# tsunrise/r1cs-spartan

Measured on AMD Instinct MI355X. Metric: R1CS constraints proved/sec at 2^20, higher is better.
Workload: dtype bls12-381 Fr/Fq Montgomery (u32 limbs)

## Files before the change

r1cs-spartan_amd/csrc/msm_common.hip:

```cpp
#include "msm_common.hpp"

#include <algorithm>
#include <cmath>
#include <cstring>
#include <cstdlib>

namespace spx {

__device__ __constant__ constexpr uint32_t kFqR2[12] = {0x1c341746u, 0xf4df1f34u, 0x09d104f1u, 0x0a76e6a6u,
                                                       0x4c95b6d5u, 0x8de5476cu, 0x939d83c0u, 0x67eb88a9u,
                                                       0xb519952du, 0x9a793e85u, 0x92cae3aau, 0x11988fe5u};

struct Digits {
    uint32_t s[8];
    uint32_t carry = 0;
    DEV int32_t next(uint32_t c) {
        const uint32_t full = 1u << c, half = full >> 1;
        uint32_t v = (s[0] & (full - 1)) + carry;
#pragma unroll
        for (int k = 0; k < 7; ++k) s[k] = (s[k] >> c) | (s[k + 1] << (32 - c));
        s[7] >>= c;
        carry = v > half;
        return carry ? (int32_t)v - (int32_t)full : (int32_t)v;
    }
// ... 390 lines not shown
    if (!handoff_last(ticket, g.nbin, &last)) return;
    for (int l = 0; l <= nlev; ++l) {
        uint32_t carry = 0;
        const uint32_t* src = binsum + (size_t)l * (g.nbin + 1);
        uint32_t* dst = binpfx + (size_t)l * (g.nbin + 1);
        for (uint32_t b = 0; b < g.nbin; b += NT) {
            const uint32_t i = b + f;
            const uint32_t x = i < g.nbin ? ld_agent(src + i) : 0u;
            const uint32_t e = block_excl_scan<NT>(x, agg, L.sh);
            if (i < g.nbin) dst[i] = carry + e;
            carry += agg;
        }
        if (f == 0) dst[g.nbin] = carry;
    }
    if (f == 0) *ticket = 0u;
}

__global__ __launch_bounds__(kScanThreads) void k_sort_final(SortGeom g, int nlev, LevPtrs lev, const uint32_t* __restrict__ binpfx) {
    const uint64_t t = blockIdx.x * (uint64_t)kScanThreads + threadIdx.x;
    const uint32_t l = (uint32_t)(t / (g.nb + 1)), b = (uint32_t)(t % (g.nb + 1));
    if ((int)l > nlev) return;
    const uint32_t* pf = binpfx + (size_t)l * (g.nbin + 1);
    lev.p[l][b] = b < g.nb ? lev.p[l][b] + pf[b >> g.sb] : pf[g.nbin];
}

uint32_t seg1_len(bool) { return kSeg1Default; }

uint32_t seg1_fit(uint32_t seg1, uint64_t refs, int waves_per_simd, int lanes_per_elem) {
    static const int cus = [] {
        int dev = 0, n = 0;
        if (hipGetDevice(&dev) != hipSuccess || hipDeviceGetAttribute(&n, hipDeviceAttributeMultiprocessorCount, dev) != hipSuccess)
            n = 0;
        return n;
    }();
    if (cus <= 0 || refs == 0) return seg1;
    const uint64_t slots = (uint64_t)cus * 4 * waves_per_simd * 64 / lanes_per_elem;
    const uint64_t nthr = (refs + seg1 - 1) / seg1;
    const uint64_t rounds = (nthr + slots - 1) / slots;
    if (rounds > 16) return seg1;
    const uint64_t fit = (refs + rounds * slots - 1) / (rounds * slots);
    return (uint32_t)std::min<uint64_t>(seg1, std::max<uint64_t>(fit, std::min<uint32_t>(seg1, 8)));
}

MsmWorkspace* msm_ws_create() {
    auto* ws = new MsmWorkspace();
    ws->hot_on = msm_hot_default();
    return ws;
}
void msm_ws_destroy(MsmWorkspace* ws) { delete ws; }
void msm_ws_staging_reset(MsmWorkspace* ws) {
    if (ws) ws->pin.reset();
}
void msm_ws_note_overflow(MsmWorkspace* ws) {
    if (ws) ws->cap_scale = std::min(ws->cap_scale * 1.5, 64.0);
}
void msm_ws_set_hot(MsmWorkspace* ws, bool on) {
    if (ws) ws->hot_on = on;
}
bool msm_hot_default() {
    static const bool v = [] {
        const char* e = getenv("SPX_MSM_HOT");
        return !(e && atoi(e) == 0 && *e);
    }();
    return v;
}
uint32_t msm_hot_cap(uint64_t tot_refs, uint32_t seg1, int nlev) {
    uint64_t per = 1;
    for (int l = 0; l <= nlev; ++l) per *= kSeg;
    const uint64_t cap = tot_refs / ((per - 1) * std::max<uint32_t>(seg1, 1)) + 1;
    if (cap < tot_refs / (per * std::max<uint32_t>(seg1, 1)) + 1) throw std::runtime_error("MSM: hot-bucket list capacity");
    return (uint32_t)std::min<uint64_t>(cap, 0xffffffffu);
}

static double msm_cap_env() {
    const char* e = getenv("SPX_MSM_CAP_SCALE");
    const double v = e ? atof(e) : 1.0;
    return v > 0 ? v : 1.0;
}

MsmPlan msm_plan(const MsmInst* ih, int ninst, const MsmShard& sh, double cap_scale) {
    MsmPlan o;
    const int G = std::max(1, sh.world);
    int g = 0;
    while ((1 << g) < G) ++g;
    if ((1 << g) != G || sh.rank < 0 || sh.rank >= G) throw std::runtime_error("MSM shard: bad rank / world");
    o.compact = G > 1 && !sh.dense;
    uint64_t tot_refs = 0;
    double split_refs = 0, whole_refs = 0;
    int nsplit = 0;
    for (int i = 0; i < ninst; ++i) {
        MsmInst I = ih[i];
        if (!I.size) continue;
        if (I.c < 3 || I.c > 24) throw std::runtime_error("MSM window bits out of range");
        if (I.W < msm_windows(I.c)) throw std::runtime_error("MSM: too few windows for the window bits");
        const uint32_t lbf = I.c - 1;
        if (G > 1 && (int)lbf - g >= 2) {
            I.lb = lbf - g;
            I.lg = (uint32_t)g;
            I.sel = (uint32_t)sh.rank;
            split_refs += (double)I.size * I.W / G;
            ++nsplit;
        } else if (i % G == sh.rank) {
            I.lb = lbf;
            I.lg = 0;
            I.sel = 0;
            whole_refs += (double)I.size * I.W;
        } else {
            continue;
        }
        I.out = (uint32_t)i;
        I.bucket_off = o.nb;
        I.ref_off = (uint32_t)tot_refs;
        o.nb += 1u << I.lb;
        o.prefix.push_back(o.tot_sc);
        o.tot_sc += I.size;
        tot_refs += (uint64_t)I.size * I.W;
        o.mu_max = std::max(o.mu_max, (double)I.size * I.W / (double)(1u << lbf));
        o.any_split |= I.lg != 0;
        o.insts.push_back(I);
    }
    const int nact = (int)o.insts.size();
    o.prefix.push_back(o.tot_sc);
    if (tot_refs >= 0xffffffffull) throw std::runtime_error("MSM batch too large");
    if (o.compact) {
        const double cap = whole_refs + (split_refs + 8.0 * std::sqrt(split_refs) + 2048.0 * nsplit) * cap_scale * msm_cap_env();
        tot_refs = std::min<uint64_t>(tot_refs, (uint64_t)std::ceil(cap));
    }
    o.tot_refs = tot_refs;
    o.node_off.resize(nact);
    o.cnt.resize(nact);
    uint32_t tot_nodes = 0;
    for (int i = 0; i < nact; ++i) {
        o.node_off[i] = tot_nodes;
        const int lg = (int)o.insts[i].lb - (int)std::min<uint32_t>(kTreeChunkLog, o.insts[i].lb - 1);
        o.cnt[i] = 1u << lg;
        tot_nodes += o.cnt[i];
        o.levels = std::max(o.levels, lg);
    }
    o.wp.assign((size_t)(o.levels + 1) * (nact + 1), 0);
    o.cin.assign((size_t)(o.levels + 1) * nact, 0);
    uint32_t maxc = 1;
    for (int i = 0; i < nact; ++i) maxc = std::max(maxc, o.cnt[i]);
    o.top_from = o.levels + 1;
    for (int lv = 0; lv <= o.levels; ++lv) {
        uint64_t acc = 0;
        for (int i = 0; i < nact; ++i) {
            uint32_t nin = lv == 0 ? (o.cnt[i] * 2) : std::max(1u, o.cnt[i] >> (lv - 1));
            uint32_t nout = lv == 0 ? o.cnt[i] : std::max(1u, o.cnt[i] >> lv);
            o.cin[(size_t)lv * nact + i] = nin;
            o.wp[(size_t)lv * (nact + 1) + i] = acc;
            acc += nout;
        }
        o.wp[(size_t)lv * (nact + 1) + nact] = acc;
        if (lv >= 1 && o.top_from > o.levels && std::max(1u, maxc >> (lv - 1)) <= kTopNodes) o.top_from = lv;
    }
    return o;
}

void msm_upload_plan(MsmWorkspace* ws, MsmPlan& p, hipStream_t s) {
    const int nact = (int)p.insts.size();
    auto al = [](size_t x) { return (x + 15) & ~(size_t)15; };
    const size_t b0 = al(sizeof(MsmInst) * nact), b1 = al(8 * p.prefix.size()), b2 = al(8 * p.wp.size()),
                 b3 = al(4 * p.cin.size()), b4 = al(4 * p.node_off.size());
    std::vector<uint8_t> h(b0 + b1 + b2 + b3 + b4, 0);
    size_t o = 0;
    memcpy(h.data() + o, p.insts.data(), sizeof(MsmInst) * nact), o += b0;
    memcpy(h.data() + o, p.prefix.data(), 8 * p.prefix.size()), o += b1;
    memcpy(h.data() + o, p.wp.data(), 8 * p.wp.size()), o += b2;
    memcpy(h.data() + o, p.cin.data(), 4 * p.cin.size()), o += b3;
    memcpy(h.data() + o, p.node_off.data(), 4 * p.node_off.size());
    uint8_t* d = (uint8_t*)ws->tables.ensure(h.size());
    HIPCHK(hipMemcpyAsync(d, ws->pin.stage(h.data(), h.size()), h.size(), hipMemcpyHostToDevice, s));
    p.d_insts = (MsmInst*)d;
    p.d_prefix = (uint64_t*)(d + b0);
    p.d_wp = (uint64_t*)(d + b0 + b1);
    p.d_cin = (uint32_t*)(d + b0 + b1 + b2);
    p.d_noff = (uint32_t*)(d + b0 + b1 + b2 + b3);
}

static constexpr double kStagedRho = 6.0;
static constexpr size_t kTicketBytes = 128;
static int sort_form_env() {
    static const int v = [] {
        const char* e = getenv("SPX_SORT_FORM");
        if (!e) return -1;
        return std::string(e) == "staged" ? 1 : std::string(e) == "direct" ? 0 : -1;
    }();
    return v;
}
static SortGeom sort_geom(const MsmPlan& p, bool& staged) {
    SortGeom g;
    g.nb = p.nb;
    g.tot_sc = p.tot_sc;
    const double rho = p.tot_sc ? (double)p.tot_refs / (double)p.tot_sc : 0.0;
    staged = sort_form_env() >= 0 ? sort_form_env() == 1 : rho >= kStagedRho;
    int lnb = 0;
    while ((1ull << lnb) < p.nb) ++lnb;
    int sb = 8;
    if (staged)
        while (sb > 0 && (double)(1u << sb) * std::max(p.mu_max, 1.0) > 0.8 * kBinStage) --sb;
    else
        sb = std::min(8, std::max(0, lnb - 9));
    while (sb < 8 && ((uint64_t)p.nb + (1u << sb) - 1) >> sb > kMaxBins) ++sb;
    g.sb = (uint32_t)sb;
    g.nbin = (p.nb + (1u << g.sb) - 1) >> g.sb;
    if (g.nbin > kMaxBins) throw std::runtime_error("MSM batch: too many buckets for the sort");
    const int threads = staged ? kTileThreads : kDirectThreads, tiles_log = staged ? 8 : 9;
    const uint64_t tile_sc = (uint64_t)threads << tiles_log;
    g.spt = (uint32_t)std::min<uint64_t>(64, std::max<uint64_t>(1, (p.tot_sc + tile_sc - 1) / tile_sc));
    const uint64_t ts = (uint64_t)threads * g.spt;
    const uint64_t nt = (p.tot_sc + ts - 1) / ts;
    if (nt > 0x7fffffffull / kSub) throw std::runtime_error("MSM batch: too many tiles");
    g.ntile = (uint32_t)std::max<uint64_t>(1, nt);
    g.sub = staged ? kSub : 1;
    return g;
}

MsmSorted msm_sort(MsmWorkspace* ws, const MsmPlan& p, const Fr* scalars, void* out_dev, size_t out_bytes, hipStream_t s,
                   uint32_t seg1, int nlev) {
    if (nlev > kMaxLev) throw std::runtime_error("MSM: too many partial levels");
    if (out_bytes % 4) throw std::runtime_error("MSM: output bytes not a multiple of 4");
    MsmSorted o;
    bool staged = false;
    const SortGeom g = sort_geom(p, staged);
    const uint32_t nb = p.nb;
    const uint64_t cap = std::max<uint64_t>(p.tot_refs, 1);
    uint32_t* st = (uint32_t*)((uint8_t*)out_dev + out_bytes - 16);
    o.offs = (uint32_t*)ws->offs.ensure(4 * (size_t)(nb + 1));
    o.refs = (uint32_t*)ws->refs.ensure(4 * cap);
    uint32_t* cnt = (uint32_t*)ws->cnt.ensure(4 * (size_t)g.nbin * g.ntile * g.sub);
    uint32_t* bintot = (uint32_t*)ws->bintot.ensure(4 * (size_t)g.nbin);
    uint32_t* binbase = (uint32_t*)ws->binbase.ensure(4 * (size_t)(g.nbin + 1));
    uint32_t* binsum = (uint32_t*)ws->binsum.ensure(4 * 2 * (size_t)(kMaxLev + 1) * (g.nbin + 1));
    uint32_t* binpfx = binsum + (size_t)(kMaxLev + 1) * (g.nbin + 1);
    uint32_t* sref = (uint32_t*)ws->stage_ref.ensure(4 * cap + 16);
    uint8_t* sfine = (uint8_t*)ws->stage_fine.ensure(cap + 16);
    uint32_t* lv = (uint32_t*)ws->lvl.ensure(4 * (size_t)(nb + 1) * (nlev + 1));
    uint32_t* tk = (uint32_t*)ws->tickets.ensure(kTicketBytes);
    if (!ws->tickets_zeroed) {
        HIPCHK(hipMemsetAsync(tk, 0, kTicketBytes, s));
        ws->tickets_zeroed = true;
    }
    LevPtrs lp{};
    for (int l = 0; l <= nlev; ++l) lp.p[l] = lv + (size_t)l * (nb + 1);
    o.hot_cap = msm_hot_cap(p.tot_refs, seg1, nlev);
    o.hot = (uint32_t*)ws->hot.ensure(4 * (size_t)o.hot_cap);
    const int nact = (int)p.insts.size();
    kp_begin(KP_SORT, s);
    hipLaunchKernelGGL(k_sort_count, dim3(g.ntile * g.sub), dim3(kCountThreads), 0, s, p.d_insts, p.d_prefix, nact, scalars, g,
                       cnt, (uint32_t*)out_dev, (uint32_t)(out_bytes / 4));
    const uint32_t cap32 = (uint32_t)std::min<uint64_t>(cap, 0xffffffffu);
    if (staged) {
        hipLaunchKernelGGL(k_sort_scan<kRowThreads>, dim3(g.nbin), dim3(kRowThreads), 0, s, cnt, g, bintot, binbase, tk, cap32,
                           st, o.offs + nb);
        hipLaunchKernelGGL(k_sort_scatter, dim3(g.ntile), dim3(kTileThreads), 0, s, p.d_insts, p.d_prefix, nact, scalars, g, cnt,
                           binbase, st, sref, sfine);
        hipLaunchKernelGGL((k_sort_bins<kBinThreads, kBinStage>), dim3(g.nbin), dim3(kBinThreads), 0, s, g, binbase, st, sref,
                           sfine, o.offs, o.refs, seg1, nlev, lp, binsum, binpfx, tk + 16, o.hot, o.hot_cap);
    } else {
        hipLaunchKernelGGL(k_sort_scan<kDirectThreads>, dim3(g.nbin), dim3(kDirectThreads), 0, s, cnt, g, bintot, binbase, tk,
                           cap32, st, o.offs + nb);
        hipLaunchKernelGGL(k_sort_scatter_direct, dim3(g.ntile), dim3(kDirectThreads), 0, s, p.d_insts, p.d_prefix, nact, scalars,
                           g, cnt, binbase, st, sref, sfine);
        hipLaunchKernelGGL((k_sort_bins<kDirectThreads, 0>), dim3(g.nbin), dim3(kDirectThreads), 0, s, g, binbase, st, sref,
                           sfine, o.offs, o.refs, seg1, nlev, lp, binsum, binpfx, tk + 16, o.hot, o.hot_cap);
    }
    const uint64_t nfin = (uint64_t)(nlev + 1) * (nb + 1);
    hipLaunchKernelGGL(k_sort_final, dim3((unsigned)((nfin + kScanThreads - 1) / kScanThreads)), dim3(kScanThreads), 0, s, g,
                       nlev, lp, binpfx);
    kp_end(64.0 * p.tot_sc + 14.0 * p.tot_refs + 16.0 * g.nbin * g.ntile * g.sub, s, (double)p.tot_refs);
    o.np_off = lp.p[0];
    for (int l = 1; l <= nlev; ++l) o.lev.push_back(lp.p[l]);
    return o;
}

DEV bool fq_canon_to_mont(Fq& r, const Fq& c) {
    uint32_t br = 0;
#pragma unroll
    for (int i = 0; i < 12; ++i) {
        uint64_t d = (uint64_t)c.v[i] - kFqP[i] - br;
        br = (uint32_t)(d >> 63);
    }
    Fq r2;
#pragma unroll
    for (int i = 0; i < 12; ++i) r2.v[i] = kFqR2[i];
    fe_mul(r, c, r2);
    return br != 0;
}

template <int NF>
__global__ void k_points_from_bytes(Fq* pts, uint64_t n, int* err) {
    for (uint64_t j = blockIdx.x * (uint64_t)blockDim.x + threadIdx.x; j < n; j += (uint64_t)gridDim.x * blockDim.x) {
        Fq* p = pts + j * NF;
        Fq last;
        load_vec(last, p + NF - 1);
        const uint32_t flags = last.v[11] >> 30;
        bool ok = true;
        if (flags & 1u) {
            Fq z;
            fe_zero(z);
#pragma unroll
            for (int k = 0; k < NF; ++k) store_vec(p + k, z);
            continue;
        }
        Fq m[NF];
#pragma unroll
        for (int k = 0; k < NF; ++k) {
// ... 64 lines not shown
```

r1cs-spartan_amd/csrc/msm_common.hpp:

```cpp
#pragma once
#include <algorithm>
#include <cstring>
#include <stdexcept>
#include <string>
#include <vector>

#include "kernels.hpp"

namespace spx {

static constexpr uint32_t kSeg1Default = 64;
uint32_t seg1_len(bool g2);
uint32_t seg1_fit(uint32_t seg1, uint64_t refs, int waves_per_simd, int lanes_per_elem);
static constexpr uint32_t kSeg = 4;
static constexpr uint32_t kTreeChunkLog = 2;
static constexpr uint32_t kTopNodes = 32;
static constexpr int kLight = 256;
static constexpr int kHeavy = 64;

#define HIPCHK(x)                                                                                     \
    do {                                                                                              \
        hipError_t e_ = (x);                                                                          \
        if (e_ != hipSuccess) throw std::runtime_error(std::string("HIP error: ") + hipGetErrorString(e_) + \
                                                       " at " __FILE__ ":" + std::to_string(__LINE__)); \
    } while (0)

template <class F>
DEV bool aff_is_sentinel(const Aff<F>& a) {
    return FieldOps<F>::is_zero(a.x) && FieldOps<F>::is_zero(a.y);
}
template <class F>
DEV void aff_set_sentinel(Aff<F>& a) {
    FieldOps<F>::zero(a.x);
    FieldOps<F>::zero(a.y);
}

DEV int find_slot(const uint64_t* prefix, int n, uint64_t g) {
    int lo = 0, hi = n - 1;
    while (lo < hi) {
        int mid = (lo + hi + 1) >> 1;
        if (prefix[mid] <= g)
            lo = mid;
        else
            hi = mid - 1;
    }
    return lo;
}
DEV uint32_t find_bucket(const uint32_t* off, uint32_t nb, uint32_t s) {
    uint32_t lo = 0, hi = nb - 1;
    while (lo < hi) {
        uint32_t mid = (lo + hi + 1) >> 1;
        if (off[mid] <= s)
            lo = mid;
        else
            hi = mid - 1;
    }
    return lo;
}


struct DBuf {
    void* p = nullptr;
    size_t cap = 0;
    void* ensure(size_t bytes) {
        if (bytes > cap) {
            if (p) HIPCHK(hipFree(p));
            size_t nb = std::max(bytes, cap + cap / 2);
            HIPCHK(hipMalloc(&p, nb));
            cap = nb;
        }
        return p;
    }
    ~DBuf() {
        if (p) (void)hipFree(p);
    }
};

struct PinArena {
    static constexpr size_t kCap = 512 << 10;
    uint8_t* p = nullptr;
    size_t used = 0;
    PinArena() { HIPCHK(hipHostMalloc((void**)&p, kCap)); }
    ~PinArena() {
        if (p) (void)hipHostFree(p);
    }
    template <class T>
    T* stage(const T* src, size_t count) {
        const size_t o = (used + 255) & ~(size_t)255, b = sizeof(T) * count;
        if (o + b > kCap) throw std::runtime_error("MSM pinned staging arena exhausted");
        used = o + b;
        memcpy(p + o, src, b);
        return (T*)(p + o);
    }
    void reset() { used = 0; }
};

struct MsmWorkspace {
    DBuf tables, offs, refs, pa, pb, tree_a, tree_b;
    DBuf cnt, bintot, binbase, binsum, stage_ref, stage_fine, lvl, tickets;
    bool tickets_zeroed = false;
    DBuf hot;
    bool hot_on = true;
    double cap_scale = 1.0;
    PinArena pin;
};

struct MsmPlan {
    std::vector<MsmInst> insts;
    std::vector<uint64_t> prefix;
    uint32_t nb = 0;
    uint64_t tot_sc = 0;
    uint64_t tot_refs = 0;
    bool compact = false;
    double mu_max = 0;
    bool any_split = false;
    std::vector<uint32_t> node_off, cnt;
    int levels = 0;
    int top_from = 1;
    std::vector<uint64_t> wp;
    std::vector<uint32_t> cin;
    MsmInst* d_insts = nullptr;
    uint64_t *d_prefix = nullptr, *d_wp = nullptr;
    uint32_t *d_cin = nullptr, *d_noff = nullptr;
};
MsmPlan msm_plan(const MsmInst* ih, int ninst, const MsmShard& sh, double cap_scale);
void msm_upload_plan(MsmWorkspace* ws, MsmPlan& p, hipStream_t s);

uint32_t msm_hot_cap(uint64_t tot_refs, uint32_t seg1, int nlev);
struct MsmSorted {
    uint32_t *offs, *refs, *np_off;
    std::vector<uint32_t*> lev;
    uint32_t* hot = nullptr;
    uint32_t hot_cap = 0;
};
MsmSorted msm_sort(MsmWorkspace* ws, const MsmPlan& p, const Fr* scalars, void* out_dev, size_t out_bytes, hipStream_t s,
                   uint32_t seg1, int nlev);

}
```

r1cs-spartan_amd/csrc/msm_impl.hpp:

```cpp
#pragma once
#include "curve29.hpp"
#include "fq2pair.hpp"
#include "msm_common.hpp"

namespace spx {

template <class F>
struct Acc;
struct AffRaw {
    Fq x, y;
};
template <>
struct Acc<Fq> {
    using Pt = G1Slot;
    using T = F29;
    using TA = F29;
    static constexpr int kLanes = 1, kWaves = 1;
    static DEV void ld_raw(AffRaw& a, const G1Slot* p) { load_vec(*(Aff<Fq>*)&a, &p->p); }
    static DEV void unpack(T& x, T& y, const AffRaw& a) {
        f29_unpack(x, a.x.v);
        f29_unpack(y, a.y.v);
    }
    static DEV void ld_aff(T& x, T& y, const G1Slot* p) {
        AffRaw a;
// ... 133 lines not shown
        else
            x29_set_inf(p);
        return;
    }
    T sq;
    O::sqr(sq, S2::sel(h, P, R));
    const T sqo = S2::swap(sq);
    const T PP = S2::sel(h, sq, sqo), Tr = S2::sel(h, sqo, sq);
    T m3;
    O::mul(m3, S2::sel(h, P, U1), PP);
    const T m3o = S2::swap(m3);
    const T PPP = S2::sel(h, m3, m3o), Q = S2::sel(h, m3o, m3);
    T w, t;
    O::template sub<2>(w, Tr, PPP);
    O::add(t, Q, Q);
    O::template sub<4>(w, w, t);
    O::template reduce<8>(w);
    O::template sub<2>(t, Q, w);
    T y4, z4;
    O::mul(y4, S2::sel(h, R, Sa), S2::sel(h, t, PPP));
    O::mul(z4, S2::sel(h, ZZ12, ZZZ12), S2::sel(h, PP, PPP));
    const T y4o = S2::swap(y4), z4o = S2::swap(z4);
    O::template sub<2>(p.y, S2::sel(h, y4, y4o), S2::sel(h, y4o, y4));
    O::template reduce<4>(p.y);
    p.x = w;
    p.zz = S2::sel(h, z4, z4o);
    p.zzz = S2::sel(h, z4o, z4);
}

template <class F>
struct TreeLanes {
    static constexpr int v = 2 * Acc<F>::kLanes;
};
template <class F>
DEV void tree_add(X29<typename Acc<F>::T>& p, const X29<typename Acc<F>::T>& q) {
    x29_add_split(p, q);
}
template <class F>
DEV void tree_dbl(X29<typename Acc<F>::T>& p) {
    x29_dbl_split(p);
}
template <class F>
DEV uint64_t tree_elem() {
    return (blockIdx.x * (uint64_t)blockDim.x + threadIdx.x) / TreeLanes<F>::v;
}
template <class F>
static unsigned tree_blocks(uint64_t elems) {
    return (unsigned)((elems * TreeLanes<F>::v + kHeavy - 1) / kHeavy);
}

template <class F>
DEV uint64_t acc_elem() {
    return (blockIdx.x * (uint64_t)blockDim.x + threadIdx.x) / Acc<F>::kLanes;
}
template <class F>
static unsigned acc_blocks(uint64_t elems) {
    return (unsigned)((elems * Acc<F>::kLanes + kHeavy - 1) / kHeavy);
}

template <class F>
__global__ __launch_bounds__(kHeavy, Acc<F>::kWaves) void k_accum_aff(const uint32_t* __restrict__ off, uint32_t nb,
                                                                      const uint32_t* __restrict__ pfx,
                                                                      const uint32_t* __restrict__ refs,
                                                                      const typename Acc<F>::Pt* __restrict__ pts,
                                                                      Xyzz<F>* __restrict__ out, uint32_t seg1) {
    using A = Acc<F>;
    using T = typename A::TA;
    const uint32_t t = (uint32_t)acc_elem<F>();
    const uint32_t total = off[nb];
    uint32_t e = t * seg1;
    if (e >= total) return;
    const uint32_t end = min(e + seg1, total);
    uint32_t b = find_bucket(off, nb, e);
    uint32_t bend = off[b + 1];
    uint32_t slot = pfx[b] + (t - off[b] / seg1);
    X29<T> acc;
    x29_set_inf(acc);
    for (; e < end; ++e) {
        if (e == bend) {
            A::st(out + slot, acc);
            x29_set_inf(acc);
            do {
                ++b;
            } while (off[b + 1] <= e);
            bend = off[b + 1];
            slot = pfx[b];
        }
        const uint32_t r = refs[e];
        T px, py;
        A::ld_aff(px, py, pts + (r & 0x7fffffffu));
        if (A::aff_sentinel(px, py)) continue;
        x29_madd(acc, px, py, (r >> 31) != 0);
    }
    A::st(out + slot, acc);
}

template <class F>
__global__ __launch_bounds__(kHeavy, Acc<F>::kWaves) void k_accum_xyzz(const uint32_t* __restrict__ segoff, uint32_t nb,
                                                                       const uint32_t* __restrict__ off,
                                                                       const Xyzz<F>* __restrict__ in,
                                                                       Xyzz<F>* __restrict__ out) {
    using A = Acc<F>;
    using T = typename A::T;
    const uint32_t s = (uint32_t)tree_elem<F>();
    if (s >= segoff[nb]) return;
    const uint32_t b = find_bucket(segoff, nb, s);
    const uint32_t k = s - segoff[b];
    const uint32_t start = off[b] + k * kSeg;
    const uint32_t end = min(start + kSeg, off[b + 1]);
    X29<T> acc;
    A::ld(acc, in + start);
    for (uint32_t e = start + 1; e < end; ++e) {
        X29<T> p;
        A::ld(p, in + e);
        tree_add<F>(acc, p);
    }
    A::st(out + s, acc);
}

static constexpr int kHotThreads = 256;
static constexpr uint32_t kHotGrid = 64;
template <class F>
__global__ __launch_bounds__(kHotThreads, 1) void k_accum_hot(const uint32_t* __restrict__ hot, uint32_t cap,
                                                              uint32_t* __restrict__ st, const uint32_t* __restrict__ off,
                                                              Xyzz<F>* P) {
    using A = Acc<F>;
    using T = typename A::T;
    constexpr uint32_t kL = TreeLanes<F>::v, ngrp = kHotThreads / kL;
    const uint32_t nhot = min(st[kMsmStHot], cap);
    const uint32_t grp = threadIdx.x / kL;
    for (uint32_t h = blockIdx.x; h < nhot; h += gridDim.x) {
        const uint32_t b = hot[h];
        const uint32_t o = off[b], m = off[b + 1] - o;
        for (uint32_t s = 1; s < m; s <<= 1) {
            for (uint32_t i = 2 * s * grp; i + s < m; i += 2 * s * ngrp) {
                X29<T> a, c;
                A::ld(a, P + o + i);
                A::ld(c, P + o + i + s);
                tree_add<F>(a, c);
                A::st(P + o + i, a);
            }
            __syncthreads();
        }
        if (threadIdx.x == 0) atomicAdd(&st[kMsmStReduced], 1u);
    }
}

DEV uint32_t tree_chunk_log(uint32_t lb) { return lb - 1 < kTreeChunkLog ? lb - 1 : kTreeChunkLog; }

template <class F>
__global__ __launch_bounds__(kHeavy, Acc<F>::kWaves) void k_tree_chunk(
    const MsmInst* __restrict__ insts, const uint64_t* __restrict__ wp, int ninst, const uint32_t* __restrict__ node_off,
    const uint32_t* __restrict__ off, const Xyzz<F>* __restrict__ P,
    Xyzz<F>* __restrict__ Fo, Xyzz<F>* __restrict__ So, Xyzz<F>* __restrict__ Do, uint32_t hot_on, uint32_t* __restrict__ st) {
    using A = Acc<F>;
    const uint64_t t = tree_elem<F>();
    if (t >= wp[ninst]) return;
    const int i = find_slot(wp, ninst, t);
    const uint32_t k = (uint32_t)(t - wp[i]);
    const MsmInst I = insts[i];
    const uint32_t lgm = tree_chunk_log(I.lb);
    const uint32_t b0 = I.bucket_off + (k << lgm);
    const uint32_t o = node_off[i] + k;
    using T = typename A::T;
    X29<T> run;
    x29_set_inf(run);
    const int m = 1 << lgm;
    int j = m - 1;
    auto partials = [&](int jj) {
        uint32_t n = off[b0 + jj + 1] - off[b0 + jj];
        if (hot_on && n > kSeg) n = 1;
        if (n > 1 && threadIdx.x % TreeLanes<F>::v == 0 &&
            n > __hip_atomic_load(&st[kMsmStLeafMax], __ATOMIC_RELAXED, __HIP_MEMORY_SCOPE_AGENT))
            atomicMax(&st[kMsmStLeafMax], n);
        return n;
    };
    uint32_t u = 0, nu = partials(j);
#pragma unroll 1
    for (;;) {
        const bool bucket_step = u < nu;
        X29<T> a, b;
        if (bucket_step) {
            a = run;
            A::ld(b, P + off[b0 + j] + u);
            ++u;
        } else if (j == m - 1) {
            A::st(Fo + o, run);
            if (j == 0) break;
            --j;
            u = 0;
            nu = partials(j);
            continue;
        } else {
            A::ld(a, Fo + o);
            b = run;
        }
        tree_add<F>(a, b);
        if (bucket_step) {
            run = a;
        } else {
            A::st(Fo + o, a);
            if (j == 0) break;
            --j;
            u = 0;
            nu = partials(j);
        }
    }
    A::st(So + o, run);
#pragma unroll 1
    for (uint32_t d = 0; d < lgm; ++d) tree_dbl<F>(run);
    A::st(Do + o, run);
}

template <class F>
__global__ __launch_bounds__(kHeavy, Acc<F>::kWaves) void k_tree_level(
    const uint64_t* __restrict__ wp, int ninst, const uint32_t* __restrict__ node_off, const uint32_t* __restrict__ cnt_in,
    const Xyzz<F>* __restrict__ Fi, const Xyzz<F>* __restrict__ Si, const Xyzz<F>* __restrict__ Di,
    Xyzz<F>* __restrict__ Fo, Xyzz<F>* __restrict__ So, Xyzz<F>* __restrict__ Do) {
    using A = Acc<F>;
    const uint64_t t = tree_elem<F>();
    const uint64_t N = wp[ninst];
    if (t >= 3 * N) return;
    const uint32_t comp = (uint32_t)(t / N);
    const uint64_t tn = t - comp * N;
    const int i = find_slot(wp, ninst, tn);
    const uint32_t k = (uint32_t)(tn - wp[i]);
    const uint32_t base = node_off[i], n = cnt_in[i];
    const bool has_r = 2 * k + 1 < n;
    X29<typename A::T> a, b;
    if (comp == 0) {
        A::ld(a, Fi + base + 2 * k);
        if (has_r) {
            A::ld(b, Di + base + 2 * k + 1);
            tree_add<F>(a, b);
            A::ld(b, Fi + base + 2 * k + 1);
            tree_add<F>(a, b);
        }
        A::st(Fo + base + k, a);
    } else if (comp == 1) {
        A::ld(a, Si + base + 2 * k);
        if (has_r) {
            A::ld(b, Si + base + 2 * k + 1);
            tree_add<F>(a, b);
        }
        A::st(So + base + k, a);
    } else {
        A::ld(a, Di + base + 2 * k);
        if (has_r) {
            A::ld(b, Di + base + 2 * k + 1);
            tree_add<F>(a, b);
            tree_dbl<F>(a);
        }
        A::st(Do + base + k, a);
    }
}

static constexpr int kTopThreads = 128;
template <class F>
__global__ __launch_bounds__(kTopThreads, 1) void k_tree_top(const MsmInst* __restrict__ insts, int nact,
                                                             const uint32_t* __restrict__ node_off,
                                                             const uint32_t* __restrict__ cin_top, int lv0, int levels,
                                                             const Xyzz<F>* __restrict__ Fi, const Xyzz<F>* __restrict__ Si,
                                                             const Xyzz<F>* __restrict__ Di, Xyzz<F>* __restrict__ out) {
    using A = Acc<F>;
    using T = typename A::T;
    using O = Ops29<T>;
    constexpr int kL = TreeLanes<F>::v;
    __shared__ Xyzz<F> buf[2][3][kTopNodes];
    const int i = blockIdx.x;
    const MsmInst I = insts[i];
    const uint32_t base = node_off[i];
    const int grp = threadIdx.x / kL, ngrp = kTopThreads / kL;
    uint32_t nin = cin_top[i];
    for (uint32_t t = threadIdx.x; t < 3 * nin; t += blockDim.x) {
        const uint32_t comp = t / nin, k = t % nin;
        const Xyzz<F>* src = comp == 0 ? Fi : (comp == 1 ? Si : Di);
        buf[0][comp][k] = src[base + k];
    }
    __syncthreads();
    int cur = 0;
    for (int lv = lv0; lv <= levels; ++lv) {
        const uint32_t nout = nin > 1 ? nin / 2 : 1;
        for (uint32_t task = grp; task < 3 * nout; task += ngrp) {
            const uint32_t comp = task / nout, k = task % nout;
            const bool has_r = 2 * k + 1 < nin;
            X29<T> a, b;
            A::ld(a, &buf[cur][comp][2 * k]);
            if (comp == 0) {
                if (has_r) {
                    A::ld(b, &buf[cur][2][2 * k + 1]);
                    tree_add<F>(a, b);
                    A::ld(b, &buf[cur][0][2 * k + 1]);
                    tree_add<F>(a, b);
                }
            } else if (has_r) {
                A::ld(b, &buf[cur][comp][2 * k + 1]);
                tree_add<F>(a, b);
                if (comp == 2) tree_dbl<F>(a);
            }
            A::st(&buf[cur ^ 1][comp][k], a);
        }
        __syncthreads();
        cur ^= 1;
        nin = nout;
    }
    if (I.lg) {
        const uint32_t k = (1u << I.lg) - 1 - I.sel;
        if (grp == 0) {
            X29<T> f;
            A::ld(f, &buf[cur][0][0]);
#pragma unroll 1
            for (uint32_t d = 0; d < I.lg; ++d) tree_dbl<F>(f);
            A::st(&buf[cur][0][0], f);
        } else if (grp == 1 && k) {
            X29<T> sv, acc;
            A::ld(sv, &buf[cur][1][0]);
            acc = sv;
#pragma unroll 1
            for (int b = 30 - __clz(k); b >= 0; --b) {
                tree_dbl<F>(acc);
                if ((k >> b) & 1u) tree_add<F>(acc, sv);
            }
            T z;
            O::zero(z);
            O::template sub<2>(acc.y, z, acc.y);
            A::st(&buf[cur][1][1], acc);
        }
        __syncthreads();
        if (grp == 0 && k) {
            X29<T> f, acc;
            A::ld(f, &buf[cur][0][0]);
            A::ld(acc, &buf[cur][1][1]);
            tree_add<F>(f, acc);
            A::st(&buf[cur][0][0], f);
        }
    }
    __syncthreads();
    if (threadIdx.x == 0) {
        using T1 = typename R29<F>::T;
        X29<T1> a, b;
        ld29<F>(a, &buf[cur][0][0]);
        f29_map(b.x, a.x, Q29::TO_R1);
        f29_map(b.y, a.y, Q29::TO_R1);
        f29_map(b.zz, a.zz, Q29::TO_R1);
        f29_map(b.zzz, a.zzz, Q29::TO_R1);
        st29<F>(out + I.out, b);
    }
}

static int msm_levels_env() {
    static const int v = [] {
        const char* e = getenv("SPX_MSM_LEVELS");
        return e ? atoi(e) : -1;
    }();
    return v;
}
static int msm_seg1_env() {
    static const int v = [] {
        const char* e = getenv("SPX_MSM_SEG1");
        return e ? atoi(e) : 0;
    }();
    return v;
}

template <class F>
static void msm_run_t(MsmWorkspace* ws, const MsmInst* ih, int ninst, const typename Acc<F>::Pt* pts, const Fr* scalars,
                      void* out_dev, hipStream_t s, const MsmShard& sh) {
    if (ninst <= 0) return;
    const bool g2 = sizeof(F) == sizeof(Fq2);
    const size_t psz = sizeof(Xyzz<F>);
    const size_t ob = msm_out_bytes(g2, ninst);
    MsmPlan pl = msm_plan(ih, ninst, sh, ws->cap_scale);
    const int nact = (int)pl.insts.size();
    if (!nact) {
        HIPCHK(hipMemsetAsync(out_dev, 0, ob, s));
        return;
    }
    msm_upload_plan(ws, pl, s);
    const uint32_t nb = pl.nb;
    const uint64_t tot_refs = pl.tot_refs;
    uint32_t kSeg1 = seg1_fit(seg1_len(g2), tot_refs, Acc<F>::kWaves, Acc<F>::kLanes);
    if (msm_seg1_env() > 0) kSeg1 = std::min<uint32_t>(kSeg1, (uint32_t)msm_seg1_env());
    const double mu = pl.mu_max;
    int nlev = 0;
    for (uint32_t m = (uint32_t)std::ceil((mu + 6.0 * std::sqrt(mu) + 16.0) / kSeg1) + 1; m > 1; m = (m + kSeg - 1) / kSeg)
        ++nlev;
    if (msm_levels_env() >= 0) nlev = std::min(nlev, msm_levels_env());
    MsmSorted so = msm_sort(ws, pl, scalars, out_dev, ob, s, kSeg1, nlev);
    const uint64_t max_segs = tot_refs / kSeg1 + nb + 1;
    auto* PA = (Xyzz<F>*)ws->pa.ensure(psz * max_segs);
    auto* PB = (Xyzz<F>*)ws->pb.ensure(psz * (max_segs / kSeg + nb + 1));
    uint32_t* cur_off = so.np_off;
    uint32_t* nxt_off = nullptr;
    const uint64_t nthr = (tot_refs + kSeg1 - 1) / kSeg1;
    kp_begin(g2 ? KP_ACC_G2 : KP_ACC_G1, s);
    hipLaunchKernelGGL(k_accum_aff<F>, dim3(acc_blocks<F>(nthr)), dim3(kHeavy), 0, s, so.offs, nb, cur_off, so.refs, pts, PA,
                       kSeg1);
    kp_end((double)tot_refs * (4.0 + sizeof(Aff<F>)) + (double)(tot_refs / kSeg1) * psz, s, (double)tot_refs);
    Xyzz<F>* cur = PA;
    Xyzz<F>* nxt = PB;
    uint64_t cur_max_segs = max_segs;
    for (int l = 0; l < nlev; ++l) {
        nxt_off = so.lev[l];
        uint64_t nsegs = cur_max_segs / kSeg + nb + 1;
        kp_begin(g2 ? KP_ACCX_G2 : KP_ACCX_G1, s);
        hipLaunchKernelGGL(k_accum_xyzz<F>, dim3(tree_blocks<F>(nsegs)), dim3(kHeavy), 0, s, nxt_off, nb, cur_off, cur, nxt);
        kp_end((double)(cur_max_segs + nsegs) * psz, s, (double)cur_max_segs);
        std::swap(cur, nxt);
        std::swap(cur_off, nxt_off);
        cur_max_segs = nsegs;
    }
    uint32_t* stw = (uint32_t*)((uint8_t*)out_dev + ob - 16);
    if (ws->hot_on) {
        kp_begin(g2 ? KP_ACCX_G2 : KP_ACCX_G1, s);
        hipLaunchKernelGGL(k_accum_hot<F>, dim3(std::min(so.hot_cap, kHotGrid)), dim3(kHotThreads), 0, s, so.hot, so.hot_cap,
                           stw, cur_off, cur);
        kp_end(0.0, s);
    }
    uint32_t tot_nodes = 0;
    for (int i = 0; i < nact; ++i) tot_nodes += pl.cnt[i];
    auto* TA = (Xyzz<F>*)ws->tree_a.ensure(3 * psz * std::max<uint32_t>(tot_nodes, 1));
    auto* TB = (Xyzz<F>*)ws->tree_b.ensure(3 * psz * std::max<uint32_t>(tot_nodes, 1));
    Xyzz<F>* A3[3] = {TA, TA + tot_nodes, TA + 2 * (size_t)tot_nodes};
    Xyzz<F>* B3[3] = {TB, TB + tot_nodes, TB + 2 * (size_t)tot_nodes};
    kp_begin(g2 ? KP_RED_G2 : KP_RED_G1, s);
    {
        uint64_t work = pl.wp[nact];
        hipLaunchKernelGGL(k_tree_chunk<F>, dim3(tree_blocks<F>(work)), dim3(kHeavy), 0, s, pl.d_insts, pl.d_wp, nact,
                           pl.d_noff, cur_off, cur, A3[0], A3[1], A3[2], ws->hot_on ? 1u : 0u, stw);
    }
    for (int lv = 1; lv < pl.top_from; ++lv) {
        uint64_t work = 3 * pl.wp[(size_t)lv * (nact + 1) + nact];
        hipLaunchKernelGGL(k_tree_level<F>, dim3(tree_blocks<F>(work)), dim3(kHeavy), 0, s,
                           pl.d_wp + (size_t)lv * (nact + 1), nact, pl.d_noff, pl.d_cin + (size_t)lv * nact, A3[0], A3[1],
                           A3[2], B3[0], B3[1], B3[2]);
        std::swap(A3, B3);
    }
    hipLaunchKernelGGL(k_tree_top<F>, dim3(nact), dim3(kTopThreads), 0, s, pl.d_insts, nact, pl.d_noff,
                       pl.d_cin + (size_t)pl.top_from * nact, pl.top_from, pl.levels, A3[0], A3[1], A3[2],
                       (Xyzz<F>*)out_dev);
    kp_end((double)nb * psz, s);
    HIPCHK(hipGetLastError());
}

template <class F>
DEV void xyzz_from_aff(Xyzz<F>& r, const Aff<F>& a) {
    if (aff_is_sentinel(a)) {
        xyzz_set_inf(r);
        return;
    }
    r.x = a.x;
    r.y = a.y;
    FieldOps<F>::one(r.zz);
    FieldOps<F>::one(r.zzz);
}

template <class F>
__global__ __launch_bounds__(kHeavy) void k_precompute(const Aff<F>* __restrict__ raw, uint64_t count, int pair_sum,
                                                       int c, int W, Xyzz<F>* __restrict__ tmp) {
    const uint64_t j = blockIdx.x * (uint64_t)blockDim.x + threadIdx.x;
    if (j >= count) return;
    Xyzz<F> P;
    if (pair_sum) {
        Aff<F> a, b;
        load_vec(a, raw + 2 * j);
        load_vec(b, raw + 2 * j + 1);
        xyzz_from_aff(P, a);
        if (!aff_is_sentinel(b)) xyzz_madd(P, b, false);
    } else {
        Aff<F> a;
        load_vec(a, raw + j);
        xyzz_from_aff(P, a);
    }
    for (int w = 0; w < W; ++w) {
        store_vec(tmp + (uint64_t)w * count + j, P);
        if (w + 1 < W)
            for (int k = 0; k < c; ++k) xyzz_dbl(P, P);
    }
}

static constexpr int kNormChunk = 32;
template <class F>
__global__ __launch_bounds__(kHeavy) void k_normalize(const Xyzz<F>* __restrict__ in, uint64_t n, Aff<F>* __restrict__ out) {
    using O = FieldOps<F>;
    const uint64_t t = blockIdx.x * (uint64_t)blockDim.x + threadIdx.x;
    const uint64_t b = t * kNormChunk;
    if (b >= n) return;
    const uint64_t e = min(b + (uint64_t)kNormChunk, n);
    F acc;
    O::one(acc);
    for (uint64_t k = b; k < e; ++k) {
        Xyzz<F> p;
        load_vec(p, in + k);
        out[k].x = acc;
        if (!xyzz_is_inf(p)) {
            F d;
            O::mul(d, p.zz, p.zzz);
            O::mul(acc, acc, d);
        }
    }
    F inv;
    O::inv(inv, acc);
    for (uint64_t k = e; k-- > b;) {
        Xyzz<F> p;
        load_vec(p, in + k);
        if (xyzz_is_inf(p)) {
            Aff<F> a;
            aff_set_sentinel(a);
            store_vec(out + k, a);
            continue;
        }
        F d, di, izz, izzz;
        O::mul(di, inv, out[k].x);
        O::mul(d, p.zz, p.zzz);
        O::mul(inv, inv, d);
        O::mul(izz, di, p.zzz);
        O::mul(izzz, di, p.zz);
        Aff<F> a;
        O::mul(a.x, p.x, izz);
        O::mul(a.y, p.y, izzz);
        store_vec(out + k, a);
    }
}

template <class F>
__global__ __launch_bounds__(kHeavy) void k_aff_to_r29(Aff<F>* __restrict__ a, uint64_t n) {
    using T = typename R29<F>::T;
    const uint64_t j = blockIdx.x * (uint64_t)blockDim.x + threadIdx.x;
    if (j >= n) return;
    Aff<F> p;
    load_vec(p, a + j);
    T x, y, mx, my;
    R29<F>::unpack(x, p.x);
    R29<F>::unpack(y, p.y);
    f29_map(mx, x, Q29::FROM_R1);
    f29_map(my, y, Q29::FROM_R1);
    R29<F>::pack(p.x, mx);
    R29<F>::pack(p.y, my);
    store_vec(a + j, p);
}

template <class F>
static void precompute_windows_t(const Aff<F>* raw, uint64_t count, bool pair_sum, int c, int W, Aff<F>* dst, void* tmp,
                               hipStream_t s) {
    if (!count) return;
    Xyzz<F>* t = (Xyzz<F>*)tmp;
    hipLaunchKernelGGL(k_precompute<F>, dim3((unsigned)((count + kHeavy - 1) / kHeavy)), dim3(kHeavy), 0, s, raw, count,
                       pair_sum ? 1 : 0, c, W, t);
    const uint64_t n = count * (uint64_t)W;
    const uint64_t nt = (n + kNormChunk - 1) / kNormChunk;
    hipLaunchKernelGGL(k_normalize<F>, dim3((unsigned)((nt + kHeavy - 1) / kHeavy)), dim3(kHeavy), 0, s, t, n, dst);
    hipLaunchKernelGGL(k_aff_to_r29<F>, dim3((unsigned)((n + kHeavy - 1) / kHeavy)), dim3(kHeavy), 0, s, dst, n);
    HIPCHK(hipGetLastError());
}
template <class F>
__global__ __launch_bounds__(kHeavy) void k_fixed_base(const Aff<F>* __restrict__ table, const Fr* __restrict__ scalars,
                                                       uint64_t n, Xyzz<F>* __restrict__ tmp) {
    const uint64_t j = blockIdx.x * (uint64_t)blockDim.x + threadIdx.x;
    if (j >= n) return;
    Fr m, s;
    load_vec(m, scalars + j);
    fe_from_mont(s, m);
    Xyzz<F> acc;
    xyzz_set_inf(acc);
    for (int w = 0; w < 32; ++w) {
        const uint32_t d = (s.v[w >> 2] >> (8 * (w & 3))) & 0xffu;
        if (d) {
            Aff<F> a;
            load_vec(a, table + w * 256 + d);
            xyzz_madd(acc, a, false);
        }
    }
    store_vec(tmp + j, acc);
}
template <class F>
static void fixed_base_t(const Aff<F>* table, const Fr* scalars, uint64_t n, Aff<F>* out, void* tmp, hipStream_t s) {
    if (!n) return;
    Xyzz<F>* t = (Xyzz<F>*)tmp;
    hipLaunchKernelGGL(k_fixed_base<F>, dim3((unsigned)((n + kHeavy - 1) / kHeavy)), dim3(kHeavy), 0, s, table, scalars,
                       n, t);
    const uint64_t nt = (n + kNormChunk - 1) / kNormChunk;
    hipLaunchKernelGGL(k_normalize<F>, dim3((unsigned)((nt + kHeavy - 1) / kHeavy)), dim3(kHeavy), 0, s, t, n, out);
    HIPCHK(hipGetLastError());
}
}
```

Measured before the change: 66.40 million.

## Restructure bucket tree reduction in place without doubling component

The MSM bucket-reduction tree drops its third 'doubled' component (Do), which was built with repeated doublings per chunk and per level. Instead, per-level sums are kept in place in F and S arrays using strided indexing. The top kernel now doubles each level's partial S sum by the needed count and combines all terms in a shared-memory tree. This removes the per-chunk doublings, one of the two ping-pong buffers and a third of the level traffic, at the cost of more per-level tasks, a more complex top kernel with serial doubling chains, and a new cap on shared-memory elements.

```diff
diff --git a/r1cs-spartan_amd/csrc/msm_common.hip b/r1cs-spartan_amd/csrc/msm_common.hip
--- a/r1cs-spartan_amd/csrc/msm_common.hip
+++ b/r1cs-spartan_amd/csrc/msm_common.hip
@@ -566,7 +566,9 @@
             acc += nout;
         }
         o.wp[(size_t)lv * (nact + 1) + nact] = acc;
-        if (lv >= 1 && o.top_from > o.levels && std::max(1u, maxc >> (lv - 1)) <= kTopNodes) o.top_from = lv;
+        const uint32_t n = std::max(1u, maxc >> std::max(lv - 1, 0));
+        if (lv >= 1 && o.top_from > o.levels && n <= kTopNodes && n + (uint64_t)lv * std::max(1u, n / 2) <= kTopElems)
+            o.top_from = lv;
     }
     return o;
 }
diff --git a/r1cs-spartan_amd/csrc/msm_common.hpp b/r1cs-spartan_amd/csrc/msm_common.hpp
--- a/r1cs-spartan_amd/csrc/msm_common.hpp
+++ b/r1cs-spartan_amd/csrc/msm_common.hpp
@@ -15,6 +15,7 @@
 static constexpr uint32_t kSeg = 4;
 static constexpr uint32_t kTreeChunkLog = 2;
 static constexpr uint32_t kTopNodes = 32;
+static constexpr uint32_t kTopElems = 192;
 static constexpr int kLight = 256;
 static constexpr int kHeavy = 64;
 
@@ -96,7 +97,7 @@
 };
 
 struct MsmWorkspace {
-    DBuf tables, offs, refs, pa, pb, tree_a, tree_b;
+    DBuf tables, offs, refs, pa, pb, tree_a;
     DBuf cnt, bintot, binbase, binsum, stage_ref, stage_fine, lvl, tickets;
     bool tickets_zeroed = false;
     DBuf hot;
diff --git a/r1cs-spartan_amd/csrc/msm_impl.hpp b/r1cs-spartan_amd/csrc/msm_impl.hpp
--- a/r1cs-spartan_amd/csrc/msm_impl.hpp
+++ b/r1cs-spartan_amd/csrc/msm_impl.hpp
@@ -309,7 +309,7 @@
 __global__ __launch_bounds__(kHeavy, Acc<F>::kWaves) void k_tree_chunk(
     const MsmInst* __restrict__ insts, const uint64_t* __restrict__ wp, int ninst, const uint32_t* __restrict__ node_off,
     const uint32_t* __restrict__ off, const Xyzz<F>* __restrict__ P,
-    Xyzz<F>* __restrict__ Fo, Xyzz<F>* __restrict__ So, Xyzz<F>* __restrict__ Do, uint32_t hot_on, uint32_t* __restrict__ st) {
+    Xyzz<F>* __restrict__ Fo, Xyzz<F>* __restrict__ So, uint32_t hot_on, uint32_t* __restrict__ st) {
     using A = Acc<F>;
     const uint64_t t = tree_elem<F>();
     if (t >= wp[ninst]) return;
@@ -364,139 +364,132 @@
         }
     }
     A::st(So + o, run);
-#pragma unroll 1
-    for (uint32_t d = 0; d < lgm; ++d) tree_dbl<F>(run);
-    A::st(Do + o, run);
-}
-
-template <class F>
-__global__ __launch_bounds__(kHeavy, Acc<F>::kWaves) void k_tree_level(
-    const uint64_t* __restrict__ wp, int ninst, const uint32_t* __restrict__ node_off, const uint32_t* __restrict__ cnt_in,
-    const Xyzz<F>* __restrict__ Fi, const Xyzz<F>* __restrict__ Si, const Xyzz<F>* __restrict__ Di,
-    Xyzz<F>* __restrict__ Fo, Xyzz<F>* __restrict__ So, Xyzz<F>* __restrict__ Do) {
+}
+
+template <class F>
+__global__ __launch_bounds__(kHeavy, Acc<F>::kWaves) void k_tree_level(const uint64_t* __restrict__ wp, int ninst,
+                                                                       const uint32_t* __restrict__ node_off,
+                                                                       const uint32_t* __restrict__ cnt, uint32_t R,
+                                                                       Xyzz<F>* Fa, Xyzz<F>* Sa) {
     using A = Acc<F>;
     const uint64_t t = tree_elem<F>();
     const uint64_t N = wp[ninst];
-    if (t >= 3 * N) return;
+    if (t >= (R + 1) * N) return;
     const uint32_t comp = (uint32_t)(t / N);
     const uint64_t tn = t - comp * N;
     const int i = find_slot(wp, ninst, tn);
     const uint32_t k = (uint32_t)(tn - wp[i]);
-    const uint32_t base = node_off[i], n = cnt_in[i];
-    const bool has_r = 2 * k + 1 < n;
+    const uint32_t h = 1u << (R - 1);
+    const uint32_t x = (k << R) + (comp < 2 ? 0u : 1u << (comp - 2));
+    if (x + h >= cnt[i]) return;
+    Xyzz<F>* p = (comp == 0 ? Fa : Sa) + node_off[i] + x;
     X29<typename A::T> a, b;
-    if (comp == 0) {
-        A::ld(a, Fi + base + 2 * k);
-        if (has_r) {
-            A::ld(b, Di + base + 2 * k + 1);
-            tree_add<F>(a, b);
-            A::ld(b, Fi + base + 2 * k + 1);
-            tree_add<F>(a, b);
-        }
-        A::st(Fo + base + k, a);
-    } else if (comp == 1) {
-        A::ld(a, Si + base + 2 * k);
-        if (has_r) {
-            A::ld(b, Si + base + 2 * k + 1);
-            tree_add<F>(a, b);
-        }
-        A::st(So + base + k, a);
-    } else {
-        A::ld(a, Di + base + 2 * k);
-        if (has_r) {
-            A::ld(b, Di + base + 2 * k + 1);
-            tree_add<F>(a, b);
-            tree_dbl<F>(a);
-        }
-        A::st(Do + base + k, a);
-    }
+    A::ld(a, p);
+    A::ld(b, p + h);
+    tree_add<F>(a, b);
+    A::st(p, a);
 }
 
 static constexpr int kTopThreads = 128;
 template <class F>
 __global__ __launch_bounds__(kTopThreads, 1) void k_tree_top(const MsmInst* __restrict__ insts, int nact,
                                                              const uint32_t* __restrict__ node_off,
-                                                             const uint32_t* __restrict__ cin_top, int lv0, int levels,
+                                                             const uint32_t* __restrict__ cnt, uint32_t R0,
                                                              const Xyzz<F>* __restrict__ Fi, const Xyzz<F>* __restrict__ Si,
-                                                             const Xyzz<F>* __restrict__ Di, Xyzz<F>* __restrict__ out) {
+                                                             Xyzz<F>* __restrict__ out) {
     using A = Acc<F>;
     using T = typename A::T;
     using O = Ops29<T>;
     constexpr int kL = TreeLanes<F>::v;
-    __shared__ Xyzz<F> buf[2][3][kTopNodes];
+    constexpr uint32_t ngrp = kTopThreads / kL;
+    static_assert(ngrp >= 25, "one lane group per term of the root (c <= 24: at most 23)");
+    __shared__ Xyzz<F> buf[kTopElems];
     const int i = blockIdx.x;
     const MsmInst I = insts[i];
     const uint32_t base = node_off[i];
-    const int grp = threadIdx.x / kL, ngrp = kTopThreads / kL;
-    uint32_t nin = cin_top[i];
-    for (uint32_t t = threadIdx.x; t < 3 * nin; t += blockDim.x) {
-        const uint32_t comp = t / nin, k = t % nin;
-        const Xyzz<F>* src = comp == 0 ? Fi : (comp == 1 ? Si : Di);
-        buf[0][comp][k] = src[base + k];
-    }
+    const uint32_t grp = threadIdx.x / kL;
+    const uint32_t lgm = tree_chunk_log(I.lb), L = I.lb - lgm;
+    const uint32_t n = max(1u, cnt[i] >> R0), n2 = max(1u, n >> 1);
+    const uint32_t nu = min(R0, L), ns = 1 + nu;
+    const auto plain_src = [&](uint32_t j) { return (j == 0 ? Fi : Si + (1u << (j - 1))) + base; };
+    for (uint32_t t = threadIdx.x; t < n; t += blockDim.x) buf[t] = Si[base + (t << R0)];
+    if (n == 1)
+        for (uint32_t j = threadIdx.x; j < ns; j += blockDim.x) buf[1 + j] = *plain_src(j);
     __syncthreads();
-    int cur = 0;
-    for (int lv = lv0; lv <= levels; ++lv) {
-        const uint32_t nout = nin > 1 ? nin / 2 : 1;
-        for (uint32_t task = grp; task < 3 * nout; task += ngrp) {
+    for (uint32_t r = 1; (1u << r) <= n; ++r) {
+        const uint32_t h = 1u << (r - 1), nout = n >> r, per = r + ns;
+        for (uint32_t task = grp; task < per * nout; task += ngrp) {
             const uint32_t comp = task / nout, k = task % nout;
-            const bool has_r = 2 * k + 1 < nin;
+            uint32_t dst;
             X29<T> a, b;
-            A::ld(a, &buf[cur][comp][2 * k]);
-            if (comp == 0) {
-                if (has_r) {
-                    A::ld(b, &buf[cur][2][2 * k + 1]);
-                    tree_add<F>(a, b);
-                    A::ld(b, &buf[cur][0][2 * k + 1]);
-                    tree_add<F>(a, b);
+            if (comp < r) {
+                dst = (k << r) + (comp == 0 ? 0u : 1u << (comp - 1));
+                A::ld(a, &buf[dst]);
+                A::ld(b, &buf[dst + h]);
+            } else {
+                const uint32_t j = comp - r;
+                if (r == 1) {
+                    const Xyzz<F>* src = plain_src(j);
+                    dst = n + j * n2 + k;
+                    A::ld(a, src + ((2 * k) << R0));
+                    A::ld(b, src + ((2 * k + 1) << R0));
+                } else {
+                    dst = n + j * n2 + (k << (r - 1));
+                    A::ld(a, &buf[dst]);
+                    A::ld(b, &buf[dst + (h >> 1)]);
                 }
-            } else if (has_r) {
-                A::ld(b, &buf[cur][comp][2 * k + 1]);
-                tree_add<F>(a, b);
-                if (comp == 2) tree_dbl<F>(a);
             }
-            A::st(&buf[cur ^ 1][comp][k], a);
+            tree_add<F>(a, b);
+            A::st(&buf[dst], a);
         }
         __syncthreads();
-        cur ^= 1;
-        nin = nout;
-    }
-    if (I.lg) {
-        const uint32_t k = (1u << I.lg) - 1 - I.sel;
-        if (grp == 0) {
-            X29<T> f;
-            A::ld(f, &buf[cur][0][0]);
+    }
+    const uint32_t ks = I.lg ? (1u << I.lg) - 1 - I.sel : 0;
+    const uint32_t nterm = L + 1 + (ks ? 1 : 0);
+    X29<T> v;
+    if (grp < nterm) {
+        if (grp == L + 1) {
+            X29<T> sv;
+            A::ld(sv, &buf[0]);
+            v = sv;
 #pragma unroll 1
-            for (uint32_t d = 0; d < I.lg; ++d) tree_dbl<F>(f);
-            A::st(&buf[cur][0][0], f);
-        } else if (grp == 1 && k) {
-            X29<T> sv, acc;
-            A::ld(sv, &buf[cur][1][0]);
-            acc = sv;
-#pragma unroll 1
-            for (int b = 30 - __clz(k); b >= 0; --b) {
-                tree_dbl<F>(acc);
-                if ((k >> b) & 1u) tree_add<F>(acc, sv);
+            for (int b = 30 - __clz(ks); b >= 0; --b) {
+                tree_dbl<F>(v);
+                if ((ks >> b) & 1u) tree_add<F>(v, sv);
             }
             T z;
             O::zero(z);
-            O::template sub<2>(acc.y, z, acc.y);
-            A::st(&buf[cur][1][1], acc);
+            O::template sub<2>(v.y, z, v.y);
+        } else {
+            uint32_t src = n, nd = I.lg;
+            if (grp) {
+                const uint32_t l = grp - 1;
+                src = l < nu ? n + (1 + l) * n2 : 1u << (l - R0);
+                nd += lgm + l;
+            }
+            A::ld(v, &buf[src]);
+#pragma unroll 1
+            for (uint32_t d = 0; d < nd; ++d) tree_dbl<F>(v);
+        }
+    }
+    __syncthreads();
+    if (grp < nterm) A::st(&buf[grp], v);
+    __syncthreads();
+    for (uint32_t s = 1; s < nterm; s <<= 1) {
+        const uint32_t x = 2 * s * grp;
+        if (x + s < nterm) {
+            X29<T> a, b;
+            A::ld(a, &buf[x]);
+            A::ld(b, &buf[x + s]);
+            tree_add<F>(a, b);
+            A::st(&buf[x], a);
         }
         __syncthreads();
-        if (grp == 0 && k) {
-            X29<T> f, acc;
-            A::ld(f, &buf[cur][0][0]);
-            A::ld(acc, &buf[cur][1][1]);
-            tree_add<F>(f, acc);
-            A::st(&buf[cur][0][0], f);
-        }
-    }
-    __syncthreads();
+    }
     if (threadIdx.x == 0) {
         using T1 = typename R29<F>::T;
         X29<T1> a, b;
-        ld29<F>(a, &buf[cur][0][0]);
+        ld29<F>(a, &buf[0]);
         f29_map(b.x, a.x, Q29::TO_R1);
         f29_map(b.y, a.y, Q29::TO_R1);
         f29_map(b.zz, a.zz, Q29::TO_R1);
@@ -576,26 +569,22 @@
     }
     uint32_t tot_nodes = 0;
     for (int i = 0; i < nact; ++i) tot_nodes += pl.cnt[i];
-    auto* TA = (Xyzz<F>*)ws->tree_a.ensure(3 * psz * std::max<uint32_t>(tot_nodes, 1));
-    auto* TB = (Xyzz<F>*)ws->tree_b.ensure(3 * psz * std::max<uint32_t>(tot_nodes, 1));
-    Xyzz<F>* A3[3] = {TA, TA + tot_nodes, TA + 2 * (size_t)tot_nodes};
-    Xyzz<F>* B3[3] = {TB, TB + tot_nodes, TB + 2 * (size_t)tot_nodes};
+    auto* TF = (Xyzz<F>*)ws->tree_a.ensure(2 * psz * std::max<uint32_t>(tot_nodes, 1));
+    auto* TS = TF + tot_nodes;
+    const uint32_t* d_cnt = pl.d_cin + nact;
     kp_begin(g2 ? KP_RED_G2 : KP_RED_G1, s);
     {
         uint64_t work = pl.wp[nact];
         hipLaunchKernelGGL(k_tree_chunk<F>, dim3(tree_blocks<F>(work)), dim3(kHeavy), 0, s, pl.d_insts, pl.d_wp, nact,
-                           pl.d_noff, cur_off, cur, A3[0], A3[1], A3[2], ws->hot_on ? 1u : 0u, stw);
+                           pl.d_noff, cur_off, cur, TF, TS, ws->hot_on ? 1u : 0u, stw);
     }
     for (int lv = 1; lv < pl.top_from; ++lv) {
-        uint64_t work = 3 * pl.wp[(size_t)lv * (nact + 1) + nact];
+        uint64_t work = (uint64_t)(lv + 1) * pl.wp[(size_t)lv * (nact + 1) + nact];
         hipLaunchKernelGGL(k_tree_level<F>, dim3(tree_blocks<F>(work)), dim3(kHeavy), 0, s,
-                           pl.d_wp + (size_t)lv * (nact + 1), nact, pl.d_noff, pl.d_cin + (size_t)lv * nact, A3[0], A3[1],
-                           A3[2], B3[0], B3[1], B3[2]);
-        std::swap(A3, B3);
-    }
-    hipLaunchKernelGGL(k_tree_top<F>, dim3(nact), dim3(kTopThreads), 0, s, pl.d_insts, nact, pl.d_noff,
-                       pl.d_cin + (size_t)pl.top_from * nact, pl.top_from, pl.levels, A3[0], A3[1], A3[2],
-                       (Xyzz<F>*)out_dev);
+                           pl.d_wp + (size_t)lv * (nact + 1), nact, pl.d_noff, d_cnt, (uint32_t)lv, TF, TS);
+    }
+    hipLaunchKernelGGL(k_tree_top<F>, dim3(nact), dim3(kTopThreads), 0, s, pl.d_insts, nact, pl.d_noff, d_cnt,
+                       (uint32_t)(pl.top_from - 1), TF, TS, (Xyzz<F>*)out_dev);
     kp_end((double)nb * psz, s);
     HIPCHK(hipGetLastError());
 }
```

Result: faster. 67.98 million (median of 6 runs) (+2.4%).
